# researchmm/MM-Diffusion

Measured on AMD Instinct MI355X. Metric: denoising steps/sec (video+audio pair), 16x64x64 / 25600, higher is better.
Workload: dtype bf16; 1 GPU; BASELINE configs[1]: Landscape base model (133.68M params), DDPM p_sample, timestep_respacing=250, per-GPU batch 4, 16x3x64x64 video + 1x25600 audio; global_batch=4, parallelism=batch-sharded x1, no in-loop collective, weights=key-seeded synthetic (mm_diffusion.synth), graph_replay=True, batch_lanes=2, finite=True, ranks_seen=1

## Files before the change

### mm-diffusion_amd/csrc/mmd_gemm.hip

```cpp
#include "mmd_common.h"

struct ConvGemmParams {
  const char* A; int64_t lda;
  const char* W;
  const float* bias;
  const char* R; int64_t ldr;
  char* Y; int64_t ldy;
  int M, Cout, Cin, ntaps;
  int D0, D1, D2;
  const float* gn_a; const float* gn_b;
  int gn_act, gn_S;
  int64_t gn_rows;
  float* stats; int64_t stats_ld;
  int taps[27 * 3];
};

struct StripSkipParams {
  const char* A2; int64_t lda2;
  const char* W2;
  const float* bias2;
};

template <int BM, int BN>
__device__ __forceinline__ void epilogue_stats(const ConvGemmParams& p, float (&sum)[BM / 64][8], float (&sq)[BM / 64][8], float* sP, int m0,
// ... 581 lines not shown
      }
      compute(it % NS);
    }
    asm volatile("s_waitcnt vmcnt(0)" ::: "memory");
    __builtin_amdgcn_s_barrier();
    asm volatile("" ::: "memory");
    cur = (nit - 1) % NS;
  }
  if (p.R) {
#pragma unroll
    for (int ps = 0; ps < NPASS; ++ps) {
      const int m = m0 + e_rr + ps * RP;
      const bool ok = m < p.M && e_co < p.Cout;
#pragma unroll
      for (int h = 0; h < 8 / EPV; ++h)
        rres[ps][h] = *(const u32x4*)(ok ? p.R + ((int64_t)m * p.ldr + e_co + h * EPV) * ES : (const char*)g_zero_page);
    }
  }
  compute(cur);
  __syncthreads();
  if (p.R) {
#pragma unroll
    for (int ps = 0; ps < NPASS; ++ps)
#pragma unroll
      for (int h = 0; h < 8 / EPV; ++h) LAUNDER4(rres[ps][h]);
  }

#pragma unroll
  for (int a = 0; a < 2; ++a)
#pragma unroll
    for (int b2 = 0; b2 < 2; ++b2) {
      const int ml = wr * 64 + b2 * 32 + l31;
#pragma unroll
      for (int q = 0; q < 4; ++q) {
        const int col = wc * 64 + a * 32 + 8 * q + 4 * half;
        f32x4 v = {acc[a][b2][4 * q], acc[a][b2][4 * q + 1], acc[a][b2][4 * q + 2], acc[a][b2][4 * q + 3]};
        *(f32x4*)(sC + ml * LDC + col) = v;
      }
    }
  __syncthreads();
  float ssum[2][8], ssq[2][8];
#pragma unroll
  for (int r = 0; r < 2; ++r)
#pragma unroll
    for (int j = 0; j < 8; ++j) ssum[r][j] = ssq[r][j] = 0.f;
  if (e_co < p.Cout) {
#pragma unroll
    for (int ps = 0; ps < NPASS; ++ps) {
      const int ml = e_rr + ps * RP;
      const int m = m0 + ml;
      if (m < p.M) {
        float v[8];
        const f32x4 c0 = *(const f32x4*)(sC + ml * LDC + e_cg * 8);
        const f32x4 c1 = *(const f32x4*)(sC + ml * LDC + e_cg * 8 + 4);
#pragma unroll
        for (int j = 0; j < 4; ++j) { v[j] = c0[j] + bs[j]; v[4 + j] = c1[j] + bs[4 + j]; }
        if (p.R) {
#pragma unroll
          for (int h = 0; h < 8 / EPV; ++h) {
            float rf[EPV];
            Elt<T>::unpack(rres[ps][h], rf);
#pragma unroll
            for (int j = 0; j < EPV; ++j) v[h * EPV + j] += rf[j];
          }
        }
#pragma unroll
        for (int h = 0; h < 8 / EPV; ++h) {
          const u32x4 pk = Elt<T>::pack(v + h * EPV);
          *(u32x4*)(p.Y + ((int64_t)m * p.ldy + e_co + h * EPV) * ES) = pk;
          if (p.stats) {
            float rf[EPV];
            Elt<T>::unpack(pk, rf);
#pragma unroll
            for (int j = 0; j < EPV; ++j) { ssum[ps / (NPASS / 2)][h * EPV + j] += rf[j]; ssq[ps / (NPASS / 2)][h * EPV + j] += rf[j] * rf[j]; }
          }
        }
      }
    }
  }
  if (p.stats) {
    __syncthreads();
    epilogue_stats<128, 128>(p, ssum, ssq, sC, m0, n0, tid);
  }
}

template <typename T, bool GN>
__global__ __launch_bounds__(256, 2) void conv_gemm_halo_kernel(const ConvGemmParams p) {
  constexpr int BM = 128, BN = 128, PH = 8, PW = 16, HWD = PW + 2, HR = (PH + 2) * HWD, HG = (HR + 7) / 8, HJ = (HG + 3) / 4;
  constexpr int EPV = Elt<T>::EPV;
  constexpr int ES = 16 / EPV;
  constexpr int LDC = BN + 4;
  constexpr int A_B = HG * 8 * 128;
  constexpr int W_B = 128 * 128;
  constexpr int MAIN_B = (2 * A_B + 2 * W_B > BM * LDC * 4) ? 2 * A_B + 2 * W_B : BM * LDC * 4;
  extern __shared__ __attribute__((aligned(16))) char smem[];
  char* sA = smem;
  char* sW = smem + 2 * A_B;
  float* sC = (float*)smem;
  int* s_taps = (int*)(smem + MAIN_B);
  float* sGN = (float*)(smem + MAIN_B + 336);

  const int tid = threadIdx.x;
  const int lane = tid & 63;
  const int wave = __builtin_amdgcn_readfirstlane(tid >> 6);
  const int wc = wave & 1, wr = wave >> 1;
  const int half = lane >> 5, l31 = lane & 31;
  if (tid < p.ntaps * 3) s_taps[tid] = p.taps[tid];

  const int Nt = (p.Cout + BN - 1) / BN;
  const int nwg = gridDim.x;
  int wgid;
  {
    const int bid = blockIdx.x, q = nwg >> 3, r = nwg & 7, xcd = bid & 7;
    wgid = (xcd < r ? xcd * (q + 1) : r * (q + 1) + (xcd - r) * q) + (bid >> 3);
  }
  const int nt = wgid % Nt, mt = wgid / Nt;
  const int n0 = nt * BN;
  const int TW = p.D2 / PW, tpf = TW * (p.D1 / PH);
  const int d0 = mt / tpf, trem = mt - d0 * tpf;
  const int h0 = (trem / TW) * PH, w0 = (trem % TW) * PW;
  const int64_t mframe = (int64_t)d0 * p.D1 * p.D2;

  const int CinV = p.Cin / EPV;
  const int nchunk = CinV >> 3;
  const int64_t K = (int64_t)p.Cin * p.ntaps;
  const int nit = nchunk * p.ntaps;

  const int lrow = lane >> 3, pc = lane & 7;
  const char* h_ptr[HJ];
  bool h_ok[HJ];
#pragma unroll
  for (int j = 0; j < HJ; ++j) {
    const int g = wave + 4 * j;
    const int r = 8 * g + lrow;
    const int hr = r / HWD, hc = r - hr * HWD;
    const int hh = h0 - 1 + hr, ww = w0 - 1 + hc;
    h_ok[j] = g < HG && r < HR && (unsigned)hh < (unsigned)p.D1 && (unsigned)ww < (unsigned)p.D2;
    const int logical = pc ^ ((r >> 1) & 7);
    h_ptr[j] = p.A + ((mframe + (int64_t)hh * p.D2 + ww) * p.lda + (int64_t)logical * EPV) * ES;
  }
  const char* w_ptr[4];
  bool w_ok[4];
#pragma unroll
  for (int i = 0; i < 4; ++i) {
    const int logical = pc ^ (((8 * i + lrow) >> 1) & 7);
    const int co = n0 + wave * 32 + 8 * i + lrow;
    w_ok[i] = co < p.Cout;
    w_ptr[i] = p.W + ((int64_t)(w_ok[i] ? co : 0) * K + (int64_t)logical * EPV) * ES;
  }
  __syncthreads();

  typedef const __attribute__((address_space(1))) void* gptr_t;
  typedef __attribute__((address_space(3))) void* lptr_t;
  auto issue_w = [&](int buf, int t, int c) {
    const int64_t offW = ((int64_t)t * p.Cin + (int64_t)c * 8 * EPV) * ES;
#pragma unroll
    for (int i = 0; i < 4; ++i) {
      const char* src = w_ok[i] ? w_ptr[i] + offW : (const char*)g_zero_page;
      __builtin_amdgcn_global_load_lds((gptr_t)src, (lptr_t)(sW + buf * W_B + (wave * 32 + 8 * i) * 128), 16, 0, 0);
    }
  };
  auto issue_h = [&](int buf, int c, int j) {
    if (wave + 4 * j < HG) {
      const char* src = h_ok[j] ? h_ptr[j] + (int64_t)c * 128 : (const char*)g_zero_page;
      __builtin_amdgcn_global_load_lds((gptr_t)src, (lptr_t)(sA + buf * A_B + (wave + 4 * j) * 1024), 16, 0, 0);
    }
// ... 1043 lines not shown
template <int KS2, int GNM, int STM>
static int launch_conv1x1_strip_skip(const ConvGemmParams& p, const StripSkipParams& q, hipStream_t st) {
  constexpr int STAGE_B = (2 + KS2) * 32 * 128;
  const int rowblocks = cdiv(p.M, 128), nsplit = strip_nsplit(rowblocks, p.Cout / 32);
  const int Cs = p.Cout / nsplit;
  constexpr size_t REC_B = 2 * 4 * 2 * 32 * sizeof(float);
  const size_t lds = 2 * (size_t)STAGE_B + 2 * (size_t)((Cs + 3) & ~3) * 4 + 4 * 128 * 4 + REC_B;
  const size_t lds_max = 2 * (size_t)STAGE_B + 2 * 2048 * 4 + 4 * 128 * 4 + REC_B;
  if (lds > lds_max) return mmd_set_error(MMD_ERR_UNSUPPORTED, "gn_conv1x1_skip: %d output channels per block", Cs);
  return mmd_launch_cap<conv1x1_strip_skip_kernel<KS2, GNM, STM>>("conv1x1_strip_skip", dim3(rowblocks * nsplit), dim3(256), lds, lds_max, st, p, nsplit, q);
}

template <int KS2>
static int dispatch_conv1x1_strip_skip(const ConvGemmParams& p, const StripSkipParams& q, hipStream_t st) {
  if (p.stats)
    return p.gn_act ? launch_conv1x1_strip_skip<KS2, 2, 1>(p, q, st) : launch_conv1x1_strip_skip<KS2, 1, 1>(p, q, st);
  return p.gn_act ? launch_conv1x1_strip_skip<KS2, 2, 0>(p, q, st) : launch_conv1x1_strip_skip<KS2, 1, 0>(p, q, st);
}

template <typename T, bool GN>
static int launch_conv_gemm_halo(const ConvGemmParams& p, hipStream_t st) {
  bool taps_ok = p.ntaps <= 9;
  for (int t = 0; t < p.ntaps && taps_ok; ++t)
    taps_ok = p.taps[t * 3] == 0 && p.taps[t * 3 + 1] >= -1 && p.taps[t * 3 + 1] <= 1 && p.taps[t * 3 + 2] >= -1 && p.taps[t * 3 + 2] <= 1;
  if (!taps_ok || p.D1 % 8 != 0 || p.D2 % 16 != 0 || (int64_t)p.D0 * p.D1 * p.D2 != p.M || p.Cin % (8 * Elt<T>::EPV) != 0)
    return mmd_set_error(MMD_ERR_UNSUPPORTED, "conv_gemm tile 130 (halo): needs spatial taps (|dh|,|dw| <= 1), D1 %% 8 == 0, D2 %% 16 == 0, "
                         "full frames and Cin a multiple of one 128-byte K step");
  if (GN && (p.ntaps != 9 || p.gn_rows % ((int64_t)p.D1 * p.D2) != 0))
    return mmd_set_error(MMD_ERR_UNSUPPORTED, "conv_gemm tile 130 with fused GroupNorm: needs the nine spatial taps and slices of whole frames");
  const size_t lds = 2 * (size_t)(23 * 8 * 128) + 2 * (size_t)(128 * 128) + 336 + (GN ? 1024 : 0);
  const int grid = (p.M / 128) * cdiv(p.Cout, 128);
  return mmd_launch<conv_gemm_halo_kernel<T, GN>>("conv_gemm_halo", dim3(grid), dim3(256), lds, st, p);
}

template <bool GN>
static int launch_conv_gemm_halo16(const ConvGemmParams& p, hipStream_t st) {
  bool taps_ok = p.ntaps == 9;
  for (int t = 0; t < p.ntaps && taps_ok; ++t)
    taps_ok = p.taps[t * 3] == 0 && p.taps[t * 3 + 1] == t / 3 - 1 && p.taps[t * 3 + 2] == t % 3 - 1;
  if (!taps_ok || p.D1 % 16 != 0 || p.D2 % 16 != 0 || (int64_t)p.D0 * p.D1 * p.D2 != p.M || p.Cin % 64 != 0 ||
      ((int64_t)p.D1 * p.D2 - 1) * p.lda * 2 + (int64_t)p.Cin * 2 >= 0x7fffffffLL || (int64_t)128 * p.Cin * 9 * 2 >= 0x7fffffffLL)
    return mmd_set_error(MMD_ERR_UNSUPPORTED, "conv_gemm tile 133 (halo, 16 x 16 patches): needs the nine spatial taps in row-major (dh, dw) order, "
                         "D1 %% 16 == 0, D2 %% 16 == 0, full frames, Cin %% 64 == 0 and frames below 2 GB");
  if (GN && p.gn_rows % ((int64_t)p.D1 * p.D2) != 0)
    return mmd_set_error(MMD_ERR_UNSUPPORTED, "conv_gemm tile 133 with fused GroupNorm: needs slices of whole frames");
  constexpr size_t OPS_B = 2 * (size_t)(41 * 8 * 128) + 3 * (size_t)(128 * 128), C_B = 256 * 132 * sizeof(float);
  const size_t lds = (OPS_B > C_B ? OPS_B : C_B) + 1024 + 256;
  const int grid = (p.M / 256) * cdiv(p.Cout, 128);
  return mmd_launch<conv_gemm_halo16_kernel<GN>>("conv_gemm_halo16", dim3(grid), dim3(512), lds, st, p);
}

template <typename T>
static bool glds_desc_ok(const ConvGemmParams& p) {
  static const bool on = mmd_env_char("MMD_GEMM_DESC") != '0';
  constexpr int ES = 16 / Elt<T>::EPV;
  int maxshift = 0;
  for (int t = 0; t < p.ntaps; ++t) {
    const int64_t sh = ((int64_t)p.taps[3 * t] * p.D1 * p.D2 + (int64_t)p.taps[3 * t + 1] * p.D2 + p.taps[3 * t + 2]) * p.lda * ES;
    if (sh > 0x3fffffff || sh < -0x3fffffff) return false;
    (void)maxshift;
  }
  return on && ((int64_t)p.M * p.lda + p.Cin) * ES < 0x7fffffffLL && (int64_t)128 * p.Cin * p.ntaps * ES < 0x7fffffffLL;
}

template <typename T>
static int launch_conv_gemm_glds(const ConvGemmParams& p, hipStream_t st) {
  const size_t lds = 128 * 132 * sizeof(float) + 336;
  const dim3 grid(cdiv(p.M, 128) * cdiv(p.Cout, 128));
  if (p.Cin % (8 * Elt<T>::EPV) != 0) return mmd_launch<conv_gemm_glds_kernel<T, false, 2, false>>("conv_gemm_glds", grid, dim3(256), lds, st, p);
  if (!glds_desc_ok<T>(p)) return mmd_launch<conv_gemm_glds_kernel<T, true, 2, false>>("conv_gemm_glds", grid, dim3(256), lds, st, p);
  return mmd_launch<conv_gemm_glds_kernel<T, true, 2, true>>("conv_gemm_glds", grid, dim3(256), lds, st, p);
}

template <typename T>
static int launch_conv_gemm_ring(const ConvGemmParams& p, hipStream_t st) {
  if (p.Cin % (8 * Elt<T>::EPV) != 0)
    return mmd_set_error(MMD_ERR_UNSUPPORTED, "conv_gemm tile 132 (deep ring): Cin must be a multiple of one 128-byte K step");
  const size_t lds = 8 * (size_t)(128 * 128) + 336;
  const dim3 grid(cdiv(p.M, 128) * cdiv(p.Cout, 128));
  if (!glds_desc_ok<T>(p)) return mmd_launch<conv_gemm_glds_kernel<T, true, 4, false>>("conv_gemm_ring", grid, dim3(256), lds, st, p);
  return mmd_launch<conv_gemm_glds_kernel<T, true, 4, true>>("conv_gemm_ring", grid, dim3(256), lds, st, p);
}

template <typename T, int BM, int BN, bool GN>
static int launch_conv_gemm(const ConvGemmParams& p, hipStream_t st) {
  const size_t lds_ops = 2 * (size_t)(BM + BN) * ROWB;
  const size_t lds_c = (size_t)BM * (BN + 4) * sizeof(float);
  const size_t lds = (lds_ops > lds_c ? lds_ops : lds_c) + 336 + (GN ? 16 * 256 : 0);
  const int grid = cdiv(p.M, BM) * cdiv(p.Cout, BN);
  return mmd_launch<conv_gemm_kernel<T, BM, BN, GN>>("conv_gemm", dim3(grid), dim3(256), lds, st, p);
}

template <typename T>
static int dispatch_conv_gemm(const ConvGemmParams& p, int tile, hipStream_t st) {
  if (tile == 133) {
    if constexpr (Elt<T>::EPV == 8) return p.gn_a ? launch_conv_gemm_halo16<true>(p, st) : launch_conv_gemm_halo16<false>(p, st);
    else return mmd_set_error(MMD_ERR_UNSUPPORTED, "conv_gemm tile 133: bf16 only");
  }
  if (p.gn_a) {
    if (tile == 130) {
      if constexpr (Elt<T>::EPV == 8) return launch_conv_gemm_halo<T, true>(p, st);
      else return mmd_set_error(MMD_ERR_UNSUPPORTED, "conv_gemm tile 130 with fused GroupNorm: bf16 only");
    }
    if (tile == 128) return launch_conv_gemm<T, 128, 128, true>(p, st);
    return launch_conv_gemm<T, 64, 64, true>(p, st);
  }
  if (tile == 129) return launch_conv_gemm_glds<T>(p, st);
  if (tile == 132) return launch_conv_gemm_ring<T>(p, st);
  if (tile == 130) return launch_conv_gemm_halo<T, false>(p, st);
  if (tile == 128) return launch_conv_gemm<T, 128, 128, false>(p, st);
  return launch_conv_gemm<T, 64, 64, false>(p, st);
}

static int conv_gemm_impl(int dtype, const void* A, int64_t lda, const void* W, const float* bias, const void* R, int64_t ldr,
                          void* Y, int64_t ldy, int M, int Cout, int Cin, int ntaps, const int* taps, int D0, int D1, int D2,
                          int tile, const float* gn_a, const float* gn_b, int gn_act, int gn_S, int64_t gn_rows, float* stats,
                          int64_t stats_ld, void* stream) {
  const int epv = dtype == MMD_BF16 ? 8 : 4;
  MMD_REQUIRE(dtype == MMD_BF16 || dtype == MMD_F32, "conv_gemm: bad dtype %d", dtype);
  MMD_REQUIRE(A && W && Y && M > 0 && Cout > 0 && Cin > 0, "conv_gemm: null/empty argument");
  MMD_REQUIRE(ntaps >= 1 && ntaps <= 27 && taps, "conv_gemm: ntaps %d out of [1,27]", ntaps);
  MMD_REQUIRE(Cin % epv == 0, "conv_gemm: Cin %d must be a multiple of %d", Cin, epv);
  MMD_REQUIRE(Cout % 8 == 0, "conv_gemm: Cout %d must be a multiple of 8", Cout);
  MMD_REQUIRE(lda % epv == 0 && ldy % epv == 0 && (!R || ldr % epv == 0), "conv_gemm: row strides must be 16-byte multiples");
  MMD_REQUIRE(((uintptr_t)A | (uintptr_t)W | (uintptr_t)Y | (uintptr_t)R) % 16 == 0, "conv_gemm: pointers must be 16-byte aligned");
  MMD_REQUIRE(D0 > 0 && D1 > 0 && D2 > 0, "conv_gemm: bad position dims");
  MMD_REQUIRE(!gn_a || (gn_b && (ntaps == 1 || tile == 130 || tile == 133) && gn_S > 0 && gn_rows >= 128 && (Cin <= 256 || tile == 131 || tile == 130 || tile == 133) &&
                        (int64_t)gn_S * gn_rows == M),
              "gn_conv1x1 / gn_conv_gemm: needs contiguous slices of >= 128 rows covering M, Cin <= 256 unless tile 130 / 131, taps only with tile 130 "
              "(got S=%d rows=%ld Cin=%d M=%d ntaps=%d tile=%d)", gn_S, (long)gn_rows, Cin, M, ntaps, tile);
  ConvGemmParams p;
  p.A = (const char*)A; p.lda = lda; p.W = (const char*)W; p.bias = bias;
  p.R = (const char*)R; p.ldr = ldr; p.Y = (char*)Y; p.ldy = ldy;
  p.M = M; p.Cout = Cout; p.Cin = Cin; p.ntaps = ntaps; p.D0 = D0; p.D1 = D1; p.D2 = D2;
  p.gn_a = gn_a; p.gn_b = gn_b; p.gn_act = gn_act; p.gn_S = gn_S; p.gn_rows = gn_rows;
  MMD_REQUIRE(!stats || (M % 64 == 0 && Cout % 4 == 0 && stats_ld >= Cout / 4 && tile != 130 && tile != 133 && (uintptr_t)stats % 8 == 0),
              "conv_gemm: output statistics need M %% 64 == 0, Cout %% 4 == 0, stats_ld >= Cout / 4 (quads) and a row-tiled main loop (not tiles 130 / 133)");
  p.stats = stats; p.stats_ld = stats_ld;
  for (int i = 0; i < ntaps * 3; ++i) p.taps[i] = taps[i];
  hipStream_t st = (hipStream_t)stream;
  if (tile == 0) tile = (int64_t)cdiv(M, 128) * cdiv(Cout, 128) >= 320 ? 128 : 64;
  MMD_REQUIRE(tile == 64 || tile == 128 || ((tile == 129 || tile == 132) && !gn_a) || (tile == 130 && (!gn_a || dtype == MMD_BF16)) ||
                  ((tile == 131 || tile == 133) && dtype == MMD_BF16),
              "conv_gemm: tile must be 0, 64, 128, 129 (128 direct-to-LDS), 130 (halo-tile 3x3), 131 (row strip, bf16 1x1 convs) or 132 (129 with a "
              "four-slot ring for launches of few tiles)");
  if (tile == 131) return dispatch_conv1x1_strip(p, st);
  return dtype == MMD_BF16 ? dispatch_conv_gemm<__bf16>(p, tile, st) : dispatch_conv_gemm<float>(p, tile, st);
}

extern "C" int mmd_conv_gemm(int dtype, const void* A, int64_t lda, const void* W, const float* bias, const void* R, int64_t ldr,
                             void* Y, int64_t ldy, int M, int Cout, int Cin, int ntaps, const int* taps, int D0, int D1, int D2,
                             int tile, void* stream) {
  return conv_gemm_impl(dtype, A, lda, W, bias, R, ldr, Y, ldy, M, Cout, Cin, ntaps, taps, D0, D1, D2, tile, nullptr, nullptr, 0, 0,
                        0, nullptr, 0, stream);
}

extern "C" int mmd_conv_gemm_stats(int dtype, const void* A, int64_t lda, const void* W, const float* bias, const void* R, int64_t ldr,
                                   void* Y, int64_t ldy, int M, int Cout, int Cin, int ntaps, const int* taps, int D0, int D1, int D2,
                                   int tile, float* stats, int64_t stats_ld, void* stream) {
  MMD_REQUIRE(stats, "conv_gemm_stats: null statistics buffer");
  return conv_gemm_impl(dtype, A, lda, W, bias, R, ldr, Y, ldy, M, Cout, Cin, ntaps, taps, D0, D1, D2, tile, nullptr, nullptr, 0, 0,
                        0, stats, stats_ld, stream);
}

extern "C" int mmd_gn_conv1x1(int dtype, const void* A, int64_t lda, const float* gn_a, const float* gn_b, int act, int S,
                              int64_t rows_per_slice, const void* W, const float* bias, const void* R, int64_t ldr, void* Y,
                              int64_t ldy, int M, int Cout, int Cin, int tile, void* stream) {
  static const int tap0[3] = {0, 0, 0};
  MMD_REQUIRE(gn_a && gn_b, "gn_conv1x1: null GroupNorm affine");
  return conv_gemm_impl(dtype, A, lda, W, bias, R, ldr, Y, ldy, M, Cout, Cin, 1, tap0, 1, 1, 1, tile, gn_a, gn_b, act, S,
                        rows_per_slice, nullptr, 0, stream);
}

extern "C" int mmd_gn_conv1x1_stats(int dtype, const void* A, int64_t lda, const float* gn_a, const float* gn_b, int act, int S,
                                    int64_t rows_per_slice, const void* W, const float* bias, const void* R, int64_t ldr, void* Y,
                                    int64_t ldy, int M, int Cout, int Cin, int tile, float* stats, int64_t stats_ld, void* stream) {
  static const int tap0[3] = {0, 0, 0};
  MMD_REQUIRE(gn_a && gn_b && stats, "gn_conv1x1_stats: null GroupNorm affine / statistics buffer");
  return conv_gemm_impl(dtype, A, lda, W, bias, R, ldr, Y, ldy, M, Cout, Cin, 1, tap0, 1, 1, 1, tile, gn_a, gn_b, act, S,
                        rows_per_slice, stats, stats_ld, stream);
}

extern "C" int mmd_gn_conv_gemm(int dtype, const void* A, int64_t lda, const float* gn_a, const float* gn_b, int act, int S,
                                int64_t rows_per_slice, const void* W, const float* bias, const void* R, int64_t ldr, void* Y,
                                int64_t ldy, int M, int Cout, int Cin, int ntaps, const int* taps, int D0, int D1, int D2, int tile,
                                void* stream) {
  MMD_REQUIRE(gn_a && gn_b, "gn_conv_gemm: null GroupNorm affine");
  MMD_REQUIRE(tile == 130 || tile == 133, "gn_conv_gemm: the fused input GroupNorm of a conv with taps exists on the halo tiles (130 / 133) only");
  return conv_gemm_impl(dtype, A, lda, W, bias, R, ldr, Y, ldy, M, Cout, Cin, ntaps, taps, D0, D1, D2, tile, gn_a, gn_b, act, S,
                        rows_per_slice, nullptr, 0, stream);
}


extern "C" int mmd_gn_conv1x1_skip(int dtype, const void* h, int64_t ldh, const float* gn_a, const float* gn_b, int act, int S,
                                   int64_t rows_per_slice, const void* W_out, const float* bias_out, const void* x, int64_t ldx, int K2,
                                   const void* W_skip, const float* bias_skip, void* Y, int64_t ldy, int M, int Cout, int K1, float* stats,
                                   int64_t stats_ld, void* stream) {
  MMD_REQUIRE(dtype == MMD_BF16 || dtype == MMD_F32, "gn_conv1x1_skip: bad dtype %d", dtype);
  MMD_REQUIRE(h && x && W_out && W_skip && Y && gn_a && gn_b && M > 0 && Cout > 0 && K1 > 0 && K2 > 0, "gn_conv1x1_skip: null/empty argument");
  MMD_REQUIRE(K1 % 8 == 0 && K2 % 8 == 0 && Cout % 8 == 0, "gn_conv1x1_skip: K1 %d, K2 %d, Cout %d must be multiples of 8", K1, K2, Cout);
  MMD_REQUIRE(K1 + K2 <= 512, "gn_conv1x1_skip: K1 + K2 = %d exceeds the 512 register-stationary channels of a row strip", K1 + K2);
  MMD_REQUIRE(ldh % 8 == 0 && ldx % 8 == 0 && ldy % 8 == 0 && ldh >= K1 && ldx >= K2 && ldy >= Cout, "gn_conv1x1_skip: row strides must be 16-byte multiples that cover the row");
  MMD_REQUIRE(((uintptr_t)h | (uintptr_t)x | (uintptr_t)W_out | (uintptr_t)W_skip | (uintptr_t)Y) % 16 == 0, "gn_conv1x1_skip: pointers must be 16-byte aligned");
  MMD_REQUIRE((int64_t)M * ldy * 2 < 0xffffffffLL, "gn_conv1x1_skip: output offsets must stay below 4 GB");
  MMD_REQUIRE(S > 0 && rows_per_slice > 0 && (int64_t)S * rows_per_slice == M, "gn_conv1x1_skip: needs contiguous slices covering M (got S=%d rows=%ld M=%d)", S,
              (long)rows_per_slice, M);
  MMD_REQUIRE(!stats || (M % 64 == 0 && Cout % 4 == 0 && stats_ld >= Cout / 4 && (uintptr_t)stats % 8 == 0),
              "gn_conv1x1_skip: output statistics need M %% 64 == 0 and stats_ld >= Cout / 4 (quads)");
  if (dtype != MMD_BF16 || K1 != 128 || (K2 != 256 && K2 != 384) || Cout % 32 != 0 || Cout > 2048 || rows_per_slice < 128)
    return mmd_set_error(MMD_ERR_UNSUPPORTED, "gn_conv1x1_skip: needs bf16, K1 == 128, K2 in {256, 384}, Cout %% 32 == 0, Cout <= 2048, slices of >= 128 rows "
                         "(got dtype=%d K1=%d K2=%d Cout=%d rows=%ld)", dtype, K1, K2, Cout, (long)rows_per_slice);
  ConvGemmParams p;
  p.A = (const char*)h; p.lda = ldh; p.W = (const char*)W_out; p.bias = bias_out;
  p.R = nullptr; p.ldr = 0; p.Y = (char*)Y; p.ldy = ldy;
  p.M = M; p.Cout = Cout; p.Cin = K1; p.ntaps = 1; p.D0 = p.D1 = p.D2 = 1;
  p.gn_a = gn_a; p.gn_b = gn_b; p.gn_act = act; p.gn_S = S; p.gn_rows = rows_per_slice;
  p.stats = stats; p.stats_ld = stats_ld;
  p.taps[0] = p.taps[1] = p.taps[2] = 0;
  StripSkipParams q;
  q.A2 = (const char*)x; q.lda2 = ldx; q.W2 = (const char*)W_skip; q.bias2 = bias_skip;
  hipStream_t st = (hipStream_t)stream;
  return K2 == 256 ? dispatch_conv1x1_strip_skip<4>(p, q, st) : dispatch_conv1x1_strip_skip<6>(p, q, st);
}
```

### mm-diffusion_amd/mm_diffusion/ops.py

```python
import contextlib
import os

import torch

from . import _hip as H

GN_EPS = 1e-5

_recorder = None
_keep = None


class recording:
    def __init__(self, plan, keep=None):
        self.plan, self.keep = plan, keep

    def __enter__(self):
        global _recorder, _keep
        self._prev, _recorder = (_recorder, _keep), self.plan
        _keep = self.keep
        return self.plan

    def __exit__(self, *a):
        global _recorder, _keep
# ... 258 lines not shown
                                 ref.view(torch.int16 if ref.element_size() == 2 else torch.int32)):
                raise H.MMDError(f"GEMM tile {tile} is not bitwise equal to tile {candidates[0]} on {key}")
        t_min = None
        for _ in range(2):
            H.call("mmd_event_record", ev[0], st)
            for _ in range(5):
                launch(tile)
            H.call("mmd_event_record", ev[1], st)
            ms = ctypes.c_float()
            H.call("mmd_event_elapsed_ms", ev[0], ev[1], ctypes.byref(ms))
            t_min = ms.value if t_min is None else min(t_min, ms.value)
        if best_ms is None or t_min < best_ms:
            best, best_ms = tile, t_min
    for e in ev:
        H.lib().mmd_event_destroy(e)
    for t, keep in saved:
        t.copy_(keep)
    _tile_cache[key] = best
    return best


_HALO_MODE = os.environ.get("MMD_GEMM_HALO", "pin")
HALO_CANDIDATE = _HALO_MODE == "1"


def halo_tile_ok(x, taps, dims):
    M, Cin = x.shape
    return (len(taps) > 1 and all(t[0] == 0 and abs(t[1]) <= 1 and abs(t[2]) <= 1 for t in taps) and dims[1] % 8 == 0
            and dims[2] % 16 == 0 and dims[0] * dims[1] * dims[2] == M and Cin % (128 // x.element_size()) == 0)


_HALO16 = _flag("MMD_HALO16")


def halo_tile_code(x, taps, dims):
    return 133 if (_HALO16 and x.dtype == torch.bfloat16 and len(taps) == 9 and dims[1] % 16 == 0 and dims[2] % 16 == 0
                   and x.shape[1] >= 256 and tuple(tuple(t) for t in taps) == tuple(TAPS_SPATIAL)) else 130


def _stats_args(stats, M, Cout):
    if stats is None:
        return None, 0
    if (stats.dtype != torch.float32 or Cout % 4 or tuple(stats.shape) != (M // 64, Cout // 4, 2) or M % 64 or stats.stride(1) != 2
            or stats.stride(2) != 1):
        raise H.MMDError(f"GEMM output statistics: expected an fp32 [M/64, Cout/4, 2] view, got {tuple(stats.shape)} strides {stats.stride()}")
    return stats.data_ptr(), stats.stride(0) // 2


_HALO_MIN_PIXELS = int(os.environ.get("MMD_HALO_MIN_PIXELS", "1024"))


def halo_tile_pinned(x, taps, dims):
    return (_HALO_MODE == "pin" and x.dtype == torch.bfloat16 and len(taps) == 9 and dims[1] * dims[2] >= _HALO_MIN_PIXELS
            and halo_tile_ok(x, taps, dims))


_STRIP_MODE = os.environ.get("MMD_GEMM_STRIP", "pin")


def strip_tile_ok(x, Cout, taps=TAPS_1, stats=None, geom=None, base=False):
    M, Cin = x.shape
    K = len(taps) * Cin
    if x.dtype != torch.bfloat16 or K not in (128, 256, 384, 512) or Cin % 64:
        return False
    if len(taps) == 1 and tuple(taps[0]) != (0, 0, 0):
        return False
    rf = 2 if K <= 256 else 1
    if Cout % (32 * rf) or Cout > 2048 or (stats is not None and M % 64):
        return False
    if base and (len(taps) != 1 or K == 512 or (stats is not None and rf != 2)):
        return False
    if geom is not None and not (len(taps) == 1 and geom.covers(M) and geom.Tn >= 128 * rf):
        return False
    return True


def strip_tile_pinned(x, Cout, taps=TAPS_1, stats=None, geom=None):
    if _STRIP_MODE == "0":
        return False
    return strip_tile_ok(x, Cout, taps, stats, geom, base=_STRIP_MODE == "base")


def _tile_name(tile):
    return {129: "128glds", 130: "128halo", 131: "strip", 132: "128ring", 133: "256halo"}.get(tile, tile)


_RING_MODE = os.environ.get("MMD_GEMM_RING", "1")


def ring_tile_candidate(x, Cout, ntaps):
    M, Cin = x.shape
    kstep = 128 // x.element_size()
    return (_RING_MODE != "0" and Cin % kstep == 0 and (Cin * ntaps) // kstep >= 4
            and ((M + 127) // 128) * ((Cout + 127) // 128) <= 384)


def _chk_conv_w(op, x, w, ntaps):
    if w.dtype != x.dtype or w.shape[1] != ntaps * x.shape[1] or not w.is_contiguous():
        raise H.MMDError(f"{op}: weight {tuple(w.shape)} {w.dtype} does not match input {tuple(x.shape)} {x.dtype} x {ntaps} taps")


def _conv_meta(op, x, Cout, ntaps, tile, residual):
    M, Cin = x.shape
    es = x.element_size()
    nbytes = es * (M * Cin + M * Cout * (2 if residual is not None else 1) + Cout * Cin * ntaps) + 4 * Cout
    return (f"{op}<{'bf16' if es == 2 else 'f32'},{_tile_name(tile)}>[M={M},K={Cin * ntaps},N={Cout}]", 2 * M * Cout * Cin * ntaps, nbytes)


def conv_gemm(x, w, bias, taps=TAPS_1, dims=(1, 1, 1), residual=None, out=None, tile=0, stats=None):
    _chk2d(x)
    M, Cin = x.shape
    Cout = w.shape[0]
    _chk_conv_w("conv_gemm", x, w, len(taps))
    out = alloc(M, Cout, dtype=x.dtype, device=x.device) if out is None else out
    _chk2d(out)
    arr, nt = H.taps_array(taps)
    es = x.element_size()
    base = (H.dt_of(x), x.data_ptr(), x.stride(0), w.data_ptr(), H.ptr(bias), H.ptr(residual),
            0 if residual is None else residual.stride(0), out.data_ptr(), out.stride(0), M, Cout, Cin, nt, arr,
            int(dims[0]), int(dims[1]), int(dims[2]))
    if tile == 0 and stats is None and halo_tile_pinned(x, taps, dims):
        tile = halo_tile_code(x, taps, dims)
    if tile == 0 and strip_tile_pinned(x, Cout, taps, stats):
        tile = 131
    if tile == 0:
        cands = (128, 129) if stats is not None else (64, 128, 129) + ((130,) if HALO_CANDIDATE and halo_tile_ok(x, taps, dims) else ())
        if ring_tile_candidate(x, Cout, nt):
            cands = cands + (132,)
        tile = _pick_tile((es, M, Cin, nt, Cout, residual is not None, False, tuple(dims) if 130 in cands else None),
                          lambda t: H.call("mmd_conv_gemm", *base, t, H.stream_handle()), M, Cout, cands, out=out, scratch=(x, residual))
    meta = _conv_meta("conv_gemm", x, Cout, nt, tile, residual)
    if stats is not None:
        _dispatch("mmd_conv_gemm_stats", *base, tile, *_stats_args(stats, M, Cout), meta=meta)
    else:
        _dispatch("mmd_conv_gemm", *base, tile, meta=meta)
    return out


_STRIP_BLOCKS_RULE = int(os.environ.get("MMD_STRIP_BLOCKS_RULE", "448"))


def strip_column_split(M, K, Cout):
    rf, cc = (2, 64) if K <= 256 else (1, 32)
    rowblocks, nch, n = -(-M // (128 * rf)), Cout // cc, 1
    for d in range(1, min(nch, 16) + 1):
        if nch % d == 0:
            n = d
            if rowblocks * d >= _STRIP_BLOCKS_RULE:
                break
    return n


def gn_tiled_ok(geom: Geom, Cin, Cout):
    return geom.contiguous and geom.Tn >= 128 and Cin <= 256 and (Cout + 127) // 128 <= 2


def gn_fusable(geom: Geom, Cin, Cout, x=None, stats=None, act=False):
    if x is not None and strip_tile_pinned(x, Cout, stats=stats):
        if not strip_tile_pinned(x, Cout, stats=stats, geom=geom):
            return False
        return not (act and strip_column_split(x.shape[0], Cin, Cout) > 2)
    return gn_tiled_ok(geom, Cin, Cout)


def gn_conv1x1(x, a, b, geom: Geom, act, w, bias, residual=None, out=None, tile=0, stats=None):
    _chk2d(x)
    M, Cin = x.shape
    Cout = w.shape[0]
    _chk_conv_w("gn_conv1x1", x, w, 1)
    out = alloc(M, Cout, dtype=x.dtype, device=x.device) if out is None else out
    _chk2d(out)
    es = x.element_size()
    tiled_ok = gn_tiled_ok(geom, Cin, Cout)
    strip_ok = strip_tile_ok(x, Cout, stats=stats, geom=geom)
    if not ((tile == 131 and strip_ok) or (tile in (64, 128) and tiled_ok) or (tile == 0 and (tiled_ok or strip_ok))):
        raise H.MMDError("gn_conv1x1: needs contiguous slices of >= 128 rows, Cin <= 256 (use gn_apply + conv_gemm otherwise)")
    base = (H.dt_of(x), x.data_ptr(), x.stride(0), a.data_ptr(), b.data_ptr(), 1 if act else 0, geom.S, geom.Tn,
            w.data_ptr(), H.ptr(bias), H.ptr(residual),
            0 if residual is None else residual.stride(0), out.data_ptr(), out.stride(0), M, Cout, Cin)
    if tile == 0 and strip_tile_pinned(x, Cout, stats=stats, geom=geom):
        tile = 131
    if tile == 0 and not tiled_ok:
        raise H.MMDError("gn_conv1x1: the row-strip kernel is switched off (MMD_GEMM_STRIP) and the tiled loader cannot take this launch")
    if tile == 0:
        tile = _pick_tile((es, M, Cin, 1, Cout, residual is not None, True),
                          lambda t: H.call("mmd_gn_conv1x1", *base, t, H.stream_handle()), M, Cout,
                          candidates=(128,) if stats is not None else (64, 128), out=out, scratch=(x, residual, a, b))
    meta = _conv_meta("gn_conv1x1", x, Cout, 1, tile, residual)
    if stats is not None:
        _dispatch("mmd_gn_conv1x1_stats", *base, tile, *_stats_args(stats, M, Cout), meta=meta)
    else:
        _dispatch("mmd_gn_conv1x1", *base, tile, meta=meta)
    return out


_STRIP_K128_RF1 = os.environ.get("MMD_STRIP_K128_RF1", "1") != "0"


def skip_fusable(h, x, cout, geom: Geom, stats=None, out=None):
    if h.dtype != torch.bfloat16 or x.dtype != torch.bfloat16 or h.dim() != 2 or x.dim() != 2 or h.shape[0] != x.shape[0]:
        return False
    M, K1 = h.shape
    if K1 != 128 or x.shape[1] not in (256, 384) or cout % 32 or cout > 2048 or not _STRIP_K128_RF1:
        return False
    if not (geom.covers(M) and geom.Tn >= 16384) or (stats is not None and M % 64):
        return False
    if not strip_tile_pinned(h, cout, stats=stats, geom=geom) or not gn_fusable(geom, K1, cout, h, stats, act=True):
        return False
    ts = (h, x) + (() if out is None else (out,))
    if any(t.stride(1) != 1 or t.stride(0) % 8 or t.data_ptr() % 16 for t in ts):
        return False
# ... 692 lines not shown
```

Measured before the change: 375.0 pair-steps/s.

## Add K-deep 64x64 direct-to-LDS conv GEMM tile as autotune candidate

After: 377.7 pair-steps/s, median of 6. No clear change (+0.7%).

```diff
diff --git a/mm-diffusion_amd/csrc/mmd_gemm.hip b/mm-diffusion_amd/csrc/mmd_gemm.hip
--- a/mm-diffusion_amd/csrc/mmd_gemm.hip
+++ b/mm-diffusion_amd/csrc/mmd_gemm.hip
@@ -687,6 +687,166 @@
     __syncthreads();
     epilogue_stats<128, 128>(p, ssum, ssq, sC, m0, n0, tid);
   }
+}
+
+template <int BN, int NK>
+__device__ __forceinline__ void kdeep_compute(const char* bA, const char* bW, int half, int xsw, f32x16 (&acc)[BN / 64][1]) {
+  constexpr int TCO = BN / 64;
+  u32x4 fw[4 * NK][TCO], fa[4 * NK];
+  auto rd = [&](int s) {
+    const int phys = ((2 * (s & 3) + half) ^ xsw) * 16;
+#pragma unroll
+    for (int a = 0; a < TCO; ++a) fw[s][a] = *(const u32x4*)(bW + (s >> 2) * BN * 128 + a * 32 * 128 + phys);
+    fa[s] = *(const u32x4*)(bA + (s >> 2) * 64 * 128 + phys);
+  };
+  rd(0); rd(1);
+  FRAG_FENCE();
+#pragma unroll
+  for (int s = 0; s < 4 * NK; ++s) {
+    if (s + 2 < 4 * NK) rd(s + 2);
+#pragma unroll
+    for (int a = 0; a < TCO; ++a) Mma<__bf16>::run(fw[s][a], fa[s], acc[a][0]);
+    FRAG_FENCE();
+  }
+}
+
+template <int BN>
+__global__ __launch_bounds__(256, 2) void conv_gemm_kdeep_kernel(const ConvGemmParams p) {
+#if defined(__HIP_DEVICE_COMPILE__)
+  using T = __bf16;
+  constexpr int BM = 64, ES = 2, CPT = 8;
+  constexpr int LDC = BN + 4;
+  constexpr int A_CH = BM * 128, W_CH = BN * 128;
+  constexpr int A_ST = 2 * A_CH, W_ST = 2 * W_CH;
+  constexpr int MAIN_B = 2 * (A_ST + W_ST);
+  static_assert(MAIN_B >= BM * LDC * 4, "the fp32 staging tile overlays the ring");
+  constexpr int WI = BN / 32;
+  extern __shared__ __attribute__((aligned(16))) char smem[];
+  char* sA = smem;
+  char* sW = smem + 2 * A_ST;
+  float* sC = (float*)smem;
+  int* s_taps = (int*)(smem + MAIN_B);
+
+  const int tid = threadIdx.x;
+  const int lane = tid & 63;
+  const int wave = __builtin_amdgcn_readfirstlane(tid >> 6);
+  const int wc = wave & 1, wr = wave >> 1;
+  const int half = lane >> 5, l31 = lane & 31;
+  if (tid < p.ntaps * 3) s_taps[tid] = p.taps[tid];
+
+  const int Nt = (p.Cout + BN - 1) / BN;
+  const int nwg = gridDim.x;
+  int wgid;
+  {
+    const int bid = blockIdx.x, q = nwg >> 3, r = nwg & 7, xcd = bid & 7;
+    wgid = (xcd < r ? xcd * (q + 1) : r * (q + 1) + (xcd - r) * q) + (bid >> 3);
+  }
+  const int nt = wgid % Nt, mt = wgid / Nt;
+  const int m0 = mt * BM, n0 = nt * BN;
+
+  const int CinV = p.Cin / 8;
+  const int64_t K = (int64_t)p.Cin * p.ntaps;
+  const int nchunk = (int)(K / 64);
+  const int nst = (nchunk + 1) >> 1;
+  const int D12 = p.D1 * p.D2;
+
+  const int lrow = lane >> 3, pc = lane & 7;
+  const int c_par[2] = {pc ^ (lane >> 4), pc ^ (lane >> 4) ^ 4};
+
+  typedef __attribute__((address_space(3))) void* lptr_t;
+  const uint32_t OOB = 0xfffffff0u;
+  const int w_rows = p.Cout - n0 < BN ? p.Cout - n0 : BN;
+  const auto rsrcA = __builtin_amdgcn_make_buffer_rsrc((void*)p.A, 0, (int)(((int64_t)p.M - 1) * p.lda * ES + (int64_t)p.Cin * ES), 0x00020000);
+  const auto rsrcW = __builtin_amdgcn_make_buffer_rsrc((void*)(p.W + (int64_t)n0 * K * ES), 0, (int)((int64_t)w_rows * K * ES), 0x00020000);
+  int pp0[2], pp1[2], pp2[2];
+  uint32_t a_base[2], w_off[WI], a_voff[2][2];
+#pragma unroll
+  for (int i = 0; i < 2; ++i) {
+    const int m = m0 + wave * 16 + 8 * i + lrow;
+    if (m < p.M) {
+      pp2[i] = m % p.D2;
+      pp1[i] = (m / p.D2) % p.D1;
+      pp0[i] = (m / D12) % p.D0;
+    } else {
+      pp0[i] = pp1[i] = pp2[i] = -(1 << 28);
+    }
+    a_base[i] = (uint32_t)(((int64_t)m * p.lda + (int64_t)c_par[i] * 8) * ES);
+    a_voff[0][i] = a_voff[1][i] = OOB;
+  }
+#pragma unroll
+  for (int i = 0; i < WI; ++i) {
+    const int row = wave * (BN / 4) + 8 * i + lrow;
+    w_off[i] = row < w_rows ? (uint32_t)((row * K + (int64_t)c_par[i & 1] * 8) * ES) : OOB;
+  }
+  int u_tap[2], u_civ[2];
+  bool u_new[2] = {true, true};
+#pragma unroll
+  for (int c = 0; c < 2; ++c) { u_tap[c] = (c * CPT) / CinV; u_civ[c] = (c * CPT) % CinV; }
+  int u_k = 0;
+  __syncthreads();
+
+  auto issue = [&](int buf) {
+#pragma unroll
+    for (int c = 0; c < 2; ++c) {
+      if (u_k + c >= nchunk) break;
+      if (u_new[c]) {
+        const int t3 = u_tap[c] * 3;
+        const int o0 = __builtin_amdgcn_readfirstlane(s_taps[t3]), o1 = __builtin_amdgcn_readfirstlane(s_taps[t3 + 1]),
+                  o2 = __builtin_amdgcn_readfirstlane(s_taps[t3 + 2]);
+        const int shift = (int)((((int64_t)o0 * D12 + (int64_t)o1 * p.D2 + o2) * p.lda) * ES);
+#pragma unroll
+        for (int i = 0; i < 2; ++i) {
+          const bool ok = (unsigned)(pp0[i] + o0) < (unsigned)p.D0 && (unsigned)(pp1[i] + o1) < (unsigned)p.D1 &&
+                          (unsigned)(pp2[i] + o2) < (unsigned)p.D2;
+          a_voff[c][i] = ok ? a_base[i] + (uint32_t)shift : OOB;
+        }
+      }
+      const int soffA = u_civ[c] * 16, soffW = (u_tap[c] * p.Cin + u_civ[c] * 8) * ES;
+      char* dA = sA + buf * A_ST + c * A_CH + wave * (16 * 128);
+      char* dW = sW + buf * W_ST + c * W_CH + wave * (BN / 4 * 128);
+#pragma unroll
+      for (int i = 0; i < 2; ++i)
+        __builtin_amdgcn_raw_ptr_buffer_load_lds(rsrcA, (lptr_t)(dA + i * 1024), 16, a_voff[c][i], soffA, 0, 0);
+#pragma unroll
+      for (int i = 0; i < WI; ++i)
+        __builtin_amdgcn_raw_ptr_buffer_load_lds(rsrcW, (lptr_t)(dW + i * 1024), 16, w_off[i], soffW, 0, 0);
+    }
+    u_k += 2;
+#pragma unroll
+    for (int c = 0; c < 2; ++c) {
+      const int t = u_tap[c];
+      u_civ[c] += 2 * CPT;
+      while (u_civ[c] >= CinV) { u_civ[c] -= CinV; ++u_tap[c]; }
+      u_new[c] = u_tap[c] != t;
+    }
+  };
+
+  f32x16 acc[BN / 64][1];
+#pragma unroll
+  for (int a = 0; a < BN / 64; ++a)
+#pragma unroll
+    for (int r = 0; r < 16; ++r) acc[a][0][r] = 0.f;
+
+  const int xsw = (l31 >> 1) & 7;
+  const char* bA = sA + (wr * 32 + l31) * 128;
+  const char* bW = sW + (wc * (BN / 2) + l31) * 128;
+
+  int cur = 0;
+  issue(0);
+  asm volatile("s_waitcnt vmcnt(0)" ::: "memory");
+  __syncthreads();
+  for (int it = 0; it + 1 < nst; ++it) {
+    issue(cur ^ 1);
+    kdeep_compute<BN, 2>(bA + cur * A_ST, bW + cur * W_ST, half, xsw, acc);
+    asm volatile("s_waitcnt vmcnt(0)" ::: "memory");
+    __syncthreads();
+    cur ^= 1;
+  }
+  if (nchunk & 1) kdeep_compute<BN, 1>(bA + cur * A_ST, bW + cur * W_ST, half, xsw, acc);
+  else kdeep_compute<BN, 2>(bA + cur * A_ST, bW + cur * W_ST, half, xsw, acc);
+  __syncthreads();
+  gemm_epilogue<T, BM, BN>(p, acc, sC, m0, n0, tid, wc, wr, half, l31);
+#endif
 }
 
 template <typename T, bool GN>
@@ -1896,6 +2056,22 @@
   return mmd_launch<conv_gemm_glds_kernel<T, true, 4, true>>("conv_gemm_ring", grid, dim3(256), lds, st, p);
 }
 
+template <int BN>
+static int launch_conv_gemm_kdeep(const ConvGemmParams& p, hipStream_t st) {
+  if (p.Cin % 64 != 0) return mmd_set_error(MMD_ERR_UNSUPPORTED, "conv_gemm tile 140: Cin %d must be a multiple of 64", p.Cin);
+  if (p.gn_a) return mmd_set_error(MMD_ERR_UNSUPPORTED, "conv_gemm tile 140: no fused GroupNorm loader");
+  if (p.stats) return mmd_set_error(MMD_ERR_UNSUPPORTED, "conv_gemm tile 140: no output statistics (their records are folded in the 128-row tiles' order)");
+  for (int t = 0; t < p.ntaps; ++t) {
+    const int64_t sh = ((int64_t)p.taps[3 * t] * p.D1 * p.D2 + (int64_t)p.taps[3 * t + 1] * p.D2 + p.taps[3 * t + 2]) * p.lda * 2;
+    if (sh > 0x3fffffff || sh < -0x3fffffff) return mmd_set_error(MMD_ERR_UNSUPPORTED, "conv_gemm tile 140: tap shift beyond 1 GB");
+  }
+  if (((int64_t)p.M * p.lda + p.Cin) * 2 >= 0x7fffffffLL || (int64_t)BN * p.Cin * p.ntaps * 2 >= 0x7fffffffLL)
+    return mmd_set_error(MMD_ERR_UNSUPPORTED, "conv_gemm tile 140: activation view or weight panel of 2 GB or more");
+  const size_t lds = 4 * (size_t)(64 + BN) * 128 + 336;
+  const dim3 grid(cdiv(p.M, 64) * cdiv(p.Cout, BN));
+  return mmd_launch<conv_gemm_kdeep_kernel<BN>>("conv_gemm_kdeep", grid, dim3(256), lds, st, p);
+}
+
 template <typename T, int BM, int BN, bool GN>
 static int launch_conv_gemm(const ConvGemmParams& p, hipStream_t st) {
   const size_t lds_ops = 2 * (size_t)(BM + BN) * ROWB;
@@ -1910,6 +2086,10 @@
   if (tile == 133) {
     if constexpr (Elt<T>::EPV == 8) return p.gn_a ? launch_conv_gemm_halo16<true>(p, st) : launch_conv_gemm_halo16<false>(p, st);
     else return mmd_set_error(MMD_ERR_UNSUPPORTED, "conv_gemm tile 133: bf16 only");
+  }
+  if (tile == 140) {
+    if constexpr (Elt<T>::EPV == 8) return launch_conv_gemm_kdeep<64>(p, st);
+    else return mmd_set_error(MMD_ERR_UNSUPPORTED, "conv_gemm tile 140 (K-deep 64-row tile): bf16 only");
   }
   if (p.gn_a) {
     if (tile == 130) {
@@ -1955,9 +2135,9 @@
   hipStream_t st = (hipStream_t)stream;
   if (tile == 0) tile = (int64_t)cdiv(M, 128) * cdiv(Cout, 128) >= 320 ? 128 : 64;
   MMD_REQUIRE(tile == 64 || tile == 128 || ((tile == 129 || tile == 132) && !gn_a) || (tile == 130 && (!gn_a || dtype == MMD_BF16)) ||
-                  ((tile == 131 || tile == 133) && dtype == MMD_BF16),
-              "conv_gemm: tile must be 0, 64, 128, 129 (128 direct-to-LDS), 130 (halo-tile 3x3), 131 (row strip, bf16 1x1 convs) or 132 (129 with a "
-              "four-slot ring for launches of few tiles)");
+                  ((tile == 131 || tile == 133) && dtype == MMD_BF16) || tile == 140,
+              "conv_gemm: tile must be 0, 64, 128, 129 (128 direct-to-LDS), 130 (halo-tile 3x3), 131 (row strip, bf16 1x1 convs), 132 (129 with a "
+              "four-slot ring for launches of few tiles) or 140 (K-deep 64 x 64 direct-to-LDS tile, bf16)");
   if (tile == 131) return dispatch_conv1x1_strip(p, st);
   return dtype == MMD_BF16 ? dispatch_conv_gemm<__bf16>(p, tile, st) : dispatch_conv_gemm<float>(p, tile, st);
 }
diff --git a/mm-diffusion_amd/mm_diffusion/ops.py b/mm-diffusion_amd/mm_diffusion/ops.py
--- a/mm-diffusion_amd/mm_diffusion/ops.py
+++ b/mm-diffusion_amd/mm_diffusion/ops.py
@@ -364,7 +364,7 @@
 
 
 def _tile_name(tile):
-    return {129: "128glds", 130: "128halo", 131: "strip", 132: "128ring", 133: "256halo"}.get(tile, tile)
+    return {129: "128glds", 130: "128halo", 131: "strip", 132: "128ring", 133: "256halo", 140: "64deep"}.get(tile, tile)
 
 
 _RING_MODE = os.environ.get("MMD_GEMM_RING", "1")
@@ -374,6 +374,15 @@
     M, Cin = x.shape
     kstep = 128 // x.element_size()
     return (_RING_MODE != "0" and Cin % kstep == 0 and (Cin * ntaps) // kstep >= 4
+            and ((M + 127) // 128) * ((Cout + 127) // 128) <= 384)
+
+
+_KTILE_MODE = os.environ.get("MMD_GEMM_KTILE", "1")
+
+
+def ktile_candidate(x, Cout, ntaps):
+    M, Cin = x.shape
+    return (_KTILE_MODE != "0" and x.dtype == torch.bfloat16 and Cin % 64 == 0 and (Cin * ntaps) // 64 >= 4
             and ((M + 127) // 128) * ((Cout + 127) // 128) <= 384)
 
 
@@ -409,6 +418,8 @@
         cands = (128, 129) if stats is not None else (64, 128, 129) + ((130,) if HALO_CANDIDATE and halo_tile_ok(x, taps, dims) else ())
         if ring_tile_candidate(x, Cout, nt):
             cands = cands + (132,)
+        if stats is None and ktile_candidate(x, Cout, nt):
+            cands = cands + (140,)
         tile = _pick_tile((es, M, Cin, nt, Cout, residual is not None, False, tuple(dims) if 130 in cands else None),
                           lambda t: H.call("mmd_conv_gemm", *base, t, H.stream_handle()), M, Cout, cands, out=out, scratch=(x, residual))
     meta = _conv_meta("conv_gemm", x, Cout, nt, tile, residual)
```
